# violetdenim/c3dgs

Hardware: AMD Instinct MI355X
Metric: raster views/sec fwd+bwd @1920x1080 (higher is better)
Workload: dtype f32; 1 GPU; BASELINE.json configs[2]: synth-v1 3M Gaussians, SH deg 3, indexed-camera rasterizer (QAT inner loop), mark_visible+fwd+bwd, 1 view/step/GPU; gaussians=3000000, width=1920, height=1080, sh_codebook=304096, gaussian_codebook=754096, parallelism=replicas x1

## Files before the change

### c3dgs_amd/_lib.py

```python
import ctypes as C
import os

import torch

_HERE = os.path.dirname(os.path.abspath(__file__))
LIB_PATH = os.environ.get("C3DGS_LIB_PATH") or os.path.join(_HERE, "libc3dgs_hip.so")

_f32p = C.POINTER(C.c_float)
_i64p = C.POINTER(C.c_int64)
_i32p = C.POINTER(C.c_int32)
_u8p = C.POINTER(C.c_uint8)

RESIZE_FN = C.CFUNCTYPE(C.c_void_p, C.c_void_p, C.c_size_t)


class RasterParams(C.Structure):
    _fields_ = [
        ("P", C.c_int32), ("D", C.c_int32), ("M", C.c_int32), ("W", C.c_int32), ("H", C.c_int32),
        ("SHS", C.c_int32), ("GS", C.c_int32),
        ("background", C.c_void_p), ("means3D", C.c_void_p), ("sh", C.c_void_p), ("colors_precomp", C.c_void_p),
        ("opacities", C.c_void_p), ("scales", C.c_void_p), ("scale_factors", C.c_void_p), ("rotations", C.c_void_p),
        ("cov3D_precomp", C.c_void_p), ("sh_indices", C.c_void_p), ("g_indices", C.c_void_p),
        ("viewmatrix", C.c_void_p), ("projmatrix", C.c_void_p), ("campos", C.c_void_p),
        ("tan_fovx", C.c_float), ("tan_fovy", C.c_float), ("scale_modifier", C.c_float),
# ... 126 lines not shown
    "c3dgs_ray_fill_xyz": (C.c_int, [C.c_int32, _vp, _vp, _vp, C.c_float, C.c_int64, _vp, _vp, _vp, _vp, _vp]),
    "c3dgs_image_from_u8": (C.c_int, [C.c_int32, C.c_int32, C.c_int32, _vp, C.c_int32, _vp, C.c_int32, C.c_int32, _vp, _vp]),
    "c3dgs_adam_step": (C.c_int, [C.c_int32, C.POINTER(AdamTensor), C.c_double, C.c_double, C.c_double, _vp]),
    "c3dgs_sparse_adam_workspace_bytes": (C.c_int, [C.c_int64, C.POINTER(C.c_size_t)]),
    "c3dgs_sparse_adam_select": (C.c_int, [C.c_int64, _vp, C.c_int32, _vp, _vp]),
    "c3dgs_sparse_adam_step": (C.c_int, [C.c_int32, C.POINTER(SparseAdamTensor), C.c_int64, _vp, C.c_double, C.c_double, C.c_double,
                                         _vp]),
    "c3dgs_densify_classify": (C.c_int, [C.c_int32] + [_vp] * 7 + [C.c_float] * 4 + [_vp, _vp]),
    "c3dgs_rows_plan_workspace_bytes": (C.c_size_t, [C.c_int32]),
    "c3dgs_rows_plan": (C.c_int, [C.c_int32, _vp, C.c_int32, C.c_int64, _vp, _vp, _vp, _vp, _vp, _vp]),
    "c3dgs_rows_apply": (C.c_int, [C.c_int32, C.c_int64, _vp, _vp, _vp, C.c_int32, C.POINTER(RowsTensor), C.c_int32, C.c_int64,
                                   _vp, _vp, _vp, C.c_int32, C.c_int32, _vp]),
    "c3dgs_densify_stats": (C.c_int, [C.c_int32] + [_vp] * 7),
    "c3dgs_mcmc_workspace_bytes": (C.c_int, [C.c_int64, C.POINTER(C.c_size_t)]),
    "c3dgs_mcmc_sample": (C.c_int, [C.c_int64, _vp, _vp, C.c_int32, C.c_float, _vp, C.c_int64, _vp, C.c_int32, _vp, _vp, _vp, _vp,
                                    _vp, _vp]),
    "c3dgs_mcmc_apply": (C.c_int, [C.c_int64, C.c_int64, _vp, C.c_int64, _vp, _vp, C.c_int32, C.POINTER(RowsTensor), C.c_int32,
                                   C.c_float, _vp, _vp]),
    "c3dgs_mcmc_noise": (C.c_int, [C.c_int64] + [_vp] * 6 + [C.c_float, C.c_float, _vp]),
    "c3dgs_bilagrid_workspace_bytes": (C.c_size_t, [C.c_int32] * 5),
    "c3dgs_bilagrid_slice": (C.c_int, [C.c_int32] * 5 + [_vp] * 4),
    "c3dgs_bilagrid_slice_backward": (C.c_int, [C.c_int32] * 5 + [_vp] * 7),
    "c3dgs_bilagrid_tv": (C.c_int, [C.c_int32] * 4 + [_vp] * 4),
    "c3dgs_bilagrid_tv_backward": (C.c_int, [C.c_int32] * 4 + [_vp] * 4),
    "c3dgs_index_plan_workspace_bytes": (C.c_size_t, [C.c_int32, C.c_int32, C.c_int32]),
    "c3dgs_index_plan": (C.c_int, [C.c_int32, _vp, _vp, C.c_int32, _vp, C.c_int32, C.c_int64, C.c_int64, C.c_int64] + [_vp] * 8),
    "c3dgs_extract_rot_scale": (C.c_int, [C.c_int32, _vp, _vp, _vp, _vp]),
    "c3dgs_l1_ssim_forward": (C.c_int, [C.c_int32, C.c_int32, C.c_int32, C.c_void_p, C.c_void_p, C.c_void_p, C.c_void_p,
                                        C.c_void_p]),
    "c3dgs_l1_ssim_value": (C.c_int, [C.c_void_p, C.c_double, C.c_double, C.c_double, C.c_void_p, C.c_void_p]),
    "c3dgs_l1_ssim_backward": (C.c_int, [C.c_int32, C.c_int32, C.c_int32, C.c_void_p, C.c_void_p, C.c_void_p, C.c_void_p,
                                         C.c_float, C.c_float, C.c_void_p, C.c_void_p]),
    "c3dgs_image_metrics_ws_bytes": (C.c_size_t, [C.c_int32, C.c_int32, C.c_int32, C.c_int32]),
    "c3dgs_image_metrics": (C.c_int, [C.c_int32, C.c_int32, C.c_int32, C.c_int32, _vp, _vp, _vp, C.c_size_t, _vp, _vp]),
    "c3dgs_qat_workspace_bytes": (C.c_size_t, []),
    "c3dgs_qat_scan_bytes": (C.c_size_t, [C.c_int32]),
    "c3dgs_qat_observe": (C.c_int, [C.POINTER(QatParams), _vp, _vp]),
    "c3dgs_qat_codebooks": (C.c_int, [C.POINTER(QatParams), _vp, _vp, _vp, _vp]),
    "c3dgs_qat_codebooks_backward": (C.c_int, [C.POINTER(QatParams)] + [_vp] * 8),
    "c3dgs_qat_visible": (C.c_int, [C.POINTER(QatParams), _vp, _vp, _vp, _vp, _vp, _vp]),
    "c3dgs_qat_points": (C.c_int, [C.POINTER(QatParams)] + [_vp] * 10),
    "c3dgs_qat_points_backward": (C.c_int, [C.POINTER(QatParams)] + [_vp] * 11),
    "c3dgs_qat_quantize": (C.c_int, [C.POINTER(QatParams), C.c_int32] + [_vp] * 7),
    "c3dgs_fake_quantize": (C.c_int, [C.c_int64, _vp, _vp, C.c_int32, C.c_int32, C.c_float, _vp, _vp, _vp]),
    "c3dgs_fake_quantize_backward": (C.c_int, [C.c_int64, _vp, _vp, C.c_int32, _vp, _vp, _vp]),
    "c3dgs_debug_sort_temp_bytes": (C.c_size_t, [C.c_int32, C.c_int64, C.c_int32]),
    "c3dgs_debug_sort_pairs": (C.c_int, [C.c_int32, C.c_int64, C.c_int32, _vp, _vp, _vp, _vp, _vp, C.c_size_t, _vp]),
    "c3dgs_debug_tile_sort_temp_bytes": (C.c_size_t, [C.c_int32, C.c_int64]),
    "c3dgs_debug_tile_sort_pairs": (C.c_int, [C.c_int32, C.c_int64, _vp, _vp, _vp, _vp, _vp, C.c_size_t, _vp]),
    "c3dgs_get_geom_layout": (C.c_int, [C.c_int32, C.POINTER(GeomLayout)]),
    "c3dgs_get_binning_layout": (C.c_int, [C.c_int32, C.c_int32, C.c_int32, C.POINTER(BinningLayout)]),
    "c3dgs_get_image_layout": (C.c_int, [C.c_int32, C.c_int32, C.POINTER(ImageLayout)]),
    "c3dgs_get_compact_layout": (C.c_int, [C.c_int32, C.c_int32, C.c_int32, C.POINTER(CompactLayout)]),
    "c3dgs_get_backward_layout": (C.c_int, [C.c_int32, C.c_int32, C.POINTER(BackwardLayout)]),
    "c3dgs_backward_workspace_bytes": (C.c_size_t, [C.c_int32, C.c_int32]),
    "c3dgs_profile_enable": (C.c_int, [C.c_int]),
    "c3dgs_profile_only": (C.c_int, [C.c_char_p]),
    "c3dgs_profile_read": (C.c_int, [C.POINTER(StageTime), C.c_int]),
    "c3dgs_last_error": (C.c_char_p, []),
    "c3dgs_abi_version": (C.c_int, []),
    "c3dgs_abs_accumulate": (C.c_int, [C.c_int64, C.c_void_p, C.c_void_p, C.c_void_p]),
}
DIAG_PROTOTYPES = {
    "c3dgs_debug_lane_counters": (C.c_int, [C.POINTER(C.c_uint64), _vp]),
    "c3dgs_debug_sort_times": (C.c_int, [C.POINTER(C.c_uint64)]),
    "c3dgs_debug_gather_probe": (C.c_int, [C.c_int32, C.c_int64, _vp, _vp, _vp, _vp]),
}

_lib = None


def lib():
    global _lib
    if _lib is None:
        if not os.path.exists(LIB_PATH):
            raise RuntimeError(
                f"c3dgs_amd: {LIB_PATH} is missing. Build it with `python -m c3dgs_amd.build` "
                "(hipcc --offload-arch=gfx950). There is no CPU fallback for this package.")
        try:
            handle = C.CDLL(LIB_PATH)
        except OSError as e:
            raise RuntimeError(f"c3dgs_amd: cannot load {LIB_PATH}: {e}") from e
        diag = {n: p for n, p in DIAG_PROTOTYPES.items() if hasattr(handle, n)}
        for name, (res, args) in {**PROTOTYPES, **diag}.items():
            fn = getattr(handle, name)
            fn.restype = res
            fn.argtypes = args
        _lib = handle
    return _lib


def check(rc):
    if rc != 0:
        msg = lib().c3dgs_last_error()
        raise RuntimeError((msg or b"unknown error").decode("utf-8", "replace"))


def stream(device):
    return C.c_void_p(torch.cuda.current_stream(device).cuda_stream)


def ptr(t):
    return None if t is None else t.data_ptr()


def gpu_tensor(t, name, dtype=torch.float32):
# ... 29 lines not shown
```

### c3dgs_amd/csrc/c_abi.hip

```cpp
#include "common.hpp"
#include "mcmc.hpp"
#include "bilagrid.hpp"
#include <cfloat>
#include <climits>
#include <cstdlib>
#include <cstring>
#include <mutex>
#include <vector>

namespace c3dgs {

static thread_local std::string g_last_error;
void set_error(const std::string& msg) { g_last_error = msg; }

#define C3DGS_STAGE_TABLE(X)                                                                                                   \
    X(MARK_VISIBLE, "mark_visible") X(PREPROCESS, "preprocess") X(DEPTH_SORT, "depth_sort") X(SCAN, "scan")                    \
    X(DUPLICATE, "duplicate_with_keys") X(SORT, "sort") X(RANGES, "identify_ranges") X(RENDER_FWD, "render_forward")           \
    X(RENDER_DEPTH, "render_depth")                                                                                            \
    X(RENDER_CONTRIB, "render_contrib") X(RENDER_CONTRIB_BLEND, "render_contrib_blend") X(RENDER_CONTRIB_SUM, "render_contrib_sum") \
    X(RENDER_ERROR, "render_error") X(RENDER_ERROR_BLEND, "render_error_blend") X(RENDER_ERROR_SUM, "render_error_sum")           \
    X(ERROR_MAP_L1, "error_map_l1")                                                                                            \
    X(POSE_GRAD, "pose_grad") X(POSE_GRAD_SUMS, "pose_grad_sums") X(POSE_GRAD_FOLD, "pose_grad_fold")                          \
    X(ZERO_PARTIALS, "zero_partials") X(RENDER_BWD, "render_backward") X(BWD_PREPROCESS, "backward_preprocess")                \
    X(RENDER_DEPTH_BWD, "render_depth_backward") X(DEPTH_BWD_FOLD, "depth_backward_fold")                                      \
// ... 349 lines not shown
    for (auto& r : recs) {
        float ms = 0.f;
        if (hipEventSynchronize(r.b) == hipSuccess && hipEventElapsedTime(&ms, r.a, r.b) == hipSuccess) {
            total[r.stage] += (double)ms;
            count[r.stage]++;
        }
    }
    {
        std::lock_guard<std::mutex> lk(g_prof_mu);
        for (auto& r : recs) { g_prof_pool.push_back(r.a); g_prof_pool.push_back(r.b); }
    }
    int n = 0;
    for (int i = 0; i < ST_COUNT && n < capacity; i++) {
        if (!count[i]) continue;
        std::memset(&out[n], 0, sizeof(out[n]));
        std::strncpy(out[n].name, kStageNames[i], sizeof(out[n].name) - 1);
        out[n].total_ms = total[i];
        out[n].count = count[i];
        n++;
    }
    return n;
}
int c3dgs_abi_version(void) { return C3DGS_ABI_VERSION; }

int c3dgs_get_geom_layout(int32_t P, c3dgs_geom_layout* out)
{
    if (!out || P < 0) return fail(C3DGS_E_INVALID, "bad arguments");
    geom_layout(P, out);
    return C3DGS_OK;
}
int c3dgs_get_binning_layout(int32_t R, int32_t W, int32_t H, c3dgs_binning_layout* out)
{
    if (!out || R < 0 || W <= 0 || H <= 0) return fail(C3DGS_E_INVALID, "bad arguments");
    binning_layout(R, W, H, out);
    return C3DGS_OK;
}
int c3dgs_get_image_layout(int32_t W, int32_t H, c3dgs_image_layout* out)
{
    if (!out || W <= 0 || H <= 0) return fail(C3DGS_E_INVALID, "bad arguments");
    ImageLayout L; image_layout(W, H, &L);
    *out = L;
    return C3DGS_OK;
}
int c3dgs_get_compact_layout(int32_t R, int32_t W, int32_t H, c3dgs_compact_layout* out)
{
    if (!out || R < 0 || W <= 0 || H <= 0) return fail(C3DGS_E_INVALID, "bad arguments");
    c3dgs_binning_layout BL; binning_layout(R, W, H, &BL);
    const CompactBinLayout C = compact_bin_layout(R);
    ImageLayout IL; image_layout(W, H, &IL);
    out->cqm = BL.sort_temp + C.cqm; out->cid = BL.sort_temp + C.cid;
    out->tile_used_c = IL.tile_used_c; out->n_contrib_c = IL.n_contrib_c;
    return C3DGS_OK;
}
int c3dgs_get_backward_layout(int32_t P, int32_t R, c3dgs_backward_layout* out)
{
    if (!out || P < 0 || R < 0) return fail(C3DGS_E_INVALID, "bad arguments");
    backward_layout(P, R, out);
    return C3DGS_OK;
}
size_t c3dgs_backward_workspace_bytes(int32_t P, int32_t R)
{
    c3dgs_backward_layout L; backward_layout(P, R, &L);
    return L.total_bytes;
}

int c3dgs_mark_visible(int32_t P, const float* means3D, const float* viewmatrix, const float* projmatrix, uint8_t* present,
                       void* stream)
{
    (void)projmatrix;
    if (P < 0) return fail(C3DGS_E_INVALID, "P must be >= 0");
    if (P == 0) return C3DGS_OK;
    if (!means3D || !viewmatrix || !present) return fail(C3DGS_E_INVALID, "means3D, viewmatrix and present are required");
    C3DGS_TIMED_STAGE(ST_MARK_VISIBLE, 0, (hipStream_t)stream, launch_mark_visible(P, means3D, viewmatrix, present, (hipStream_t)stream));
    return C3DGS_OK;
}

int c3dgs_mark_visible_pose(int32_t P, const float* means3D, const float* extrinsic_vector, uint8_t* present, void* stream)
{
    if (P < 0) return fail(C3DGS_E_INVALID, "P must be >= 0");
    if (P == 0) return C3DGS_OK;
    if (!means3D || !extrinsic_vector || !present) return fail(C3DGS_E_INVALID, "means3D, extrinsic_vector and present are required");
    C3DGS_TIMED_STAGE(ST_MARK_VISIBLE, 0, (hipStream_t)stream, launch_mark_visible_pose(P, means3D, extrinsic_vector, present, (hipStream_t)stream));
    return C3DGS_OK;
}

int c3dgs_camera_from_pose(const float* extrinsic_vector, float inv_tan_half_fovx, float inv_tan_half_fovy, float* viewmatrix,
                           float* projmatrix, float* campos, void* stream)
{
    if (!extrinsic_vector || !viewmatrix || !projmatrix || !campos) return fail(C3DGS_E_INVALID, "camera_from_pose: NULL pointer");
    launch_camera_from_pose(extrinsic_vector, inv_tan_half_fovx, inv_tan_half_fovy, viewmatrix, projmatrix, campos, (hipStream_t)stream);
    C3DGS_STAGE("camera_from_pose", 0, (hipStream_t)stream);
    return C3DGS_OK;
}

int c3dgs_rasterize_gaussians(const c3dgs_raster_params* p, c3dgs_resize_fn geom_resize, void* geom_user,
                              c3dgs_resize_fn binning_resize, void* binning_user, c3dgs_resize_fn image_resize,
                              void* image_user, float* out_color, int32_t* radii, int32_t* num_rendered, void* stream)
{
    return forward_impl(p, false, geom_resize, geom_user, binning_resize, binning_user, image_resize, image_user, out_color,
                        radii, num_rendered, stream);
}

int c3dgs_rasterize_gaussians_indexed(const c3dgs_raster_params* p, c3dgs_resize_fn geom_resize, void* geom_user,
                                      c3dgs_resize_fn binning_resize, void* binning_user, c3dgs_resize_fn image_resize,
                                      void* image_user, float* out_color, int32_t* radii, int32_t* num_rendered, void* stream)
{
// ... 987 lines not shown
```

### c3dgs_amd/csrc/common.hpp

```cpp
#pragma once
#include <hip/hip_runtime.h>
#include <cstdint>
#include <cstddef>
#include <cstdio>
#include <cstring>
#include <string>

#include "../../include/c3dgs_hip.h"

namespace c3dgs {

constexpr int TILE = 16;
constexpr int TILE_PIX = 256;
constexpr int SPLAT_F4 = 3;
constexpr int PARTIAL_FLOATS = 9;
constexpr int BWD_LIST = 1024;

void set_error(const std::string& msg);
inline int fail(int code, const std::string& msg) { set_error(msg); return code; }

#define C3DGS_HIP_TRY(expr)                                                                         \
    do {                                                                                            \
        hipError_t e__ = (expr);                                                                    \
        if (e__ != hipSuccess)                                                                      \
// ... 33 lines not shown
{
    uint32_t msb = sizeof(n) * 4, step = msb;
    while (step > 1) {
        step /= 2;
        if (n >> msb) msb += step; else msb -= step;
    }
    if (n >> msb) msb++;
    return msb;
}

inline void geom_layout(int P, c3dgs_geom_layout* L)
{
    size_t o = 0, p = (size_t)(P > 0 ? P : 1);
    L->splat = o;             o = align_up(o + p * SPLAT_F4 * 16);
    L->depth_keys = o;        o = align_up(o + p * 4);
    L->depth_keys_sorted = o; o = align_up(o + p * 4);
    L->depth_order = o;       o = align_up(o + p * 4);
    L->sorted_offsets = o;    o = align_up(o + p * 8);
    L->inst_offset = o;       o = align_up(o + p * 4);
    L->rects = o;             o = align_up(o + p * 8);
    L->clamped = o;           o = align_up(o + p);
    L->block_base = o;        o = align_up(o + ((p + 255) / 256 + 2) * 4);
    L->depth_base = o;        o = align_up(o + ((p + 255) / 256 + 1) * 4);
    L->scan_temp = o;         L->scan_temp_bytes = scan_temp_bytes((int)p);
    o = align_up(o + L->scan_temp_bytes);
    L->total_bytes = o;
}

inline size_t geom_gtab_bytes(const c3dgs_raster_params& p) { return (p.g_indices && p.scales) ? align_up((size_t)(p.GS > 0 ? p.GS : 1) * 32) : 0; }

inline int tile_key_bytes_for(long long T) { return T > 65536 ? 4 : 2; }
inline int tile_key_bytes(int W, int H) { return tile_key_bytes_for((long long)tiles_x(W) * tiles_y(H)); }
inline int tile_sort_end_bit_for(long long T)
{
    const int msb = (int)higher_msb((uint32_t)T), kbits = 8 * tile_key_bytes_for(T);
    return msb < kbits ? msb : kbits;
}
inline int tile_sort_end_bit(int W, int H) { return tile_sort_end_bit_for((long long)tiles_x(W) * tiles_y(H)); }

inline void binning_layout(int R, int W, int H, c3dgs_binning_layout* L)
{
    size_t o = 0, r = (size_t)(R > 0 ? R : 1);
    const int end_bit = tile_sort_end_bit(W, H);
    const size_t kb = (size_t)tile_key_bytes(W, H);
    L->keys_unsorted = o;   o = align_up(o + r * kb);
    L->values_unsorted = o; o = align_up(o + r * 4);
    L->keys_sorted = o;     o = align_up(o + r * kb);
    L->point_list = o;      o = align_up(o + r * 4);
    L->sort_temp = o;       L->sort_temp_bytes = sort_temp_bytes((int)r, end_bit, (int)kb);
    o = align_up(o + L->sort_temp_bytes);
    L->total_bytes = o;
}

struct ImageLayout : c3dgs_image_layout { size_t tile_used_c, n_contrib_c; };
inline void image_layout(int W, int H, ImageLayout* L)
{
    size_t o = 0, n = (size_t)W * H, t = (size_t)tiles_x(W) * tiles_y(H);
    L->final_T = o;     o = align_up(o + n * 4);
    L->n_contrib = o;   o = align_up(o + n * 4);
    L->ranges = o;      o = align_up(o + t * 8);
    L->tile_used = o;   o = align_up(o + t * 4);
    L->tile_order = o;  o = align_up(o + t * 4);
    L->tile_used_c = o; o = align_up(o + t * 4);
    L->n_contrib_c = o; o = align_up(o + n * 4);
    L->total_bytes = o;
}

struct CompactBinLayout { size_t cqm, cid, bin_bytes; };
inline CompactBinLayout compact_bin_layout(int R)
{
    const size_t r = (size_t)(R > 0 ? R : 1);
    CompactBinLayout C;
    C.cqm = 0; C.cid = align_up(r); C.bin_bytes = C.cid + align_up(r * 4);
    return C;
}

inline void backward_layout(int P, int R, c3dgs_backward_layout* L)
{
    size_t o = 0, r = (size_t)(R > 0 ? R : 1), n_lists = ((size_t)(P > 0 ? P : 1) + BWD_LIST - 1) / BWD_LIST;
    L->partials = o;   o = align_up(o + r * PARTIAL_FLOATS * sizeof(float));
    L->touched = o;    o = align_up(o + r);
    L->live_ids = o;   o = align_up(o + n_lists * BWD_LIST * 4);
    L->live_slots = o; o = align_up(o + n_lists * BWD_LIST * 4);
    L->live_count = o; o = align_up(o + n_lists * 4);
    L->list_len = BWD_LIST;
    L->total_bytes = o;
}

struct DepthBackwardLayout { size_t dz, total_bytes; };
inline DepthBackwardLayout depth_backward_layout(int P, int R)
{
    c3dgs_backward_layout B; backward_layout(P, R, &B);
    const size_t r = (size_t)(R > 0 ? R : 1);
    DepthBackwardLayout L;
    L.dz = B.total_bytes;
    L.total_bytes = align_up(L.dz + r * sizeof(float));
    return L;
}

struct ContribSlot { float sum, max; uint32_t hits; };
struct ContribLayout { size_t slots, touched, touched_bytes, total_bytes; };
inline ContribLayout contrib_layout(int P, int R)
{
    (void)P;
    size_t o = 0, r = (size_t)(R > 0 ? R : 1);
    ContribLayout L;
    L.slots = o;   o = align_up(o + r * sizeof(ContribSlot));
    L.touched = o; o = align_up(o + r);
    L.touched_bytes = o - L.touched;
    L.total_bytes = o;
    return L;
}

struct ErrorLayout { size_t slots, touched, touched_bytes, total_bytes; };
inline ErrorLayout error_layout(int P, int R)
{
    (void)P;
    size_t o = 0, r = (size_t)(R > 0 ? R : 1);
    ErrorLayout L;
    L.slots = o;   o = align_up(o + r * sizeof(float));
    L.touched = o; o = align_up(o + r);
    L.touched_bytes = o - L.touched;
    L.total_bytes = o;
    return L;
}

constexpr int SPARSE_ADAM_SELECT_ROWS = 256;
struct SparseAdamLayout { size_t count, rows, block_base, total_bytes; };
inline SparseAdamLayout sparse_adam_layout(int64_t P)
{
    const size_t p = (size_t)(P > 0 ? P : 1);
    SparseAdamLayout L;
    size_t o = 0;
    L.count = o;      o = align_up(o + 4);
    L.rows = o;       o = align_up(o + p * 4);
    L.block_base = o; o = align_up(o + ((p + SPARSE_ADAM_SELECT_ROWS - 1) / SPARSE_ADAM_SELECT_ROWS + 2) * 4);
    L.total_bytes = o;
    return L;
}

struct GeomPtrs {
    float4* splat; uint32_t* depth_keys; uint32_t* depth_keys_sorted;
    uint32_t* depth_order; uint2* sorted_offsets; uint32_t* inst_offset; uint16_t* rects;
    uint8_t* clamped; uint32_t* block_base; uint32_t* depth_base; void* scan_temp; size_t scan_temp_bytes;
    float4* gtab;
};
struct BinPtrs {
    void* keys_unsorted; uint32_t* values_unsorted; void* keys_sorted; uint32_t* point_list;
    void* sort_temp; size_t sort_temp_bytes; int key_bytes;
};
struct ImgPtrs { float* final_T; uint32_t* n_contrib; uint2* ranges; uint32_t* tile_used; uint32_t* tile_order;
                 uint32_t* tile_used_c; uint32_t* n_contrib_c; };
struct CompactPtrs { uint8_t* cqm; uint32_t* cid; };
struct BwdPtrs { float* partials; uint8_t* touched; size_t touched_bytes;
                 uint32_t* live_ids; uint32_t* live_slots; uint32_t* live_count; };
struct ContribPtrs { ContribSlot* slots; uint8_t* touched; size_t touched_bytes; };
struct ErrorPtrs { float* slots; uint8_t* touched; size_t touched_bytes; };

inline GeomPtrs geom_ptrs(void* base, int P)
{
    c3dgs_geom_layout L; geom_layout(P, &L);
    char* b = (char*)base;
    return { (float4*)(b + L.splat), (uint32_t*)(b + L.depth_keys), (uint32_t*)(b + L.depth_keys_sorted), (uint32_t*)(b + L.depth_order),
             (uint2*)(b + L.sorted_offsets), (uint32_t*)(b + L.inst_offset), (uint16_t*)(b + L.rects),
             (uint8_t*)(b + L.clamped), (uint32_t*)(b + L.block_base), (uint32_t*)(b + L.depth_base), (void*)(b + L.scan_temp),
             L.scan_temp_bytes, (float4*)(b + L.total_bytes) };
}
inline BinPtrs bin_ptrs(void* base, int R, int W, int H)
{
    c3dgs_binning_layout L; binning_layout(R, W, H, &L);
    char* b = (char*)base;
    return { (void*)(b + L.keys_unsorted), (uint32_t*)(b + L.values_unsorted), (void*)(b + L.keys_sorted),
             (uint32_t*)(b + L.point_list), (void*)(b + L.sort_temp), L.sort_temp_bytes, tile_key_bytes(W, H) };
}
inline ImgPtrs img_ptrs(void* base, int W, int H)
{
    ImageLayout L; image_layout(W, H, &L);
    char* b = (char*)base;
    return { (float*)(b + L.final_T), (uint32_t*)(b + L.n_contrib), (uint2*)(b + L.ranges), (uint32_t*)(b + L.tile_used),
             (uint32_t*)(b + L.tile_order), (uint32_t*)(b + L.tile_used_c), (uint32_t*)(b + L.n_contrib_c) };
}
inline CompactPtrs compact_ptrs(const BinPtrs& bp, int R)
{
    const CompactBinLayout C = compact_bin_layout(R);
    return { (uint8_t*)bp.sort_temp + C.cqm, (uint32_t*)((char*)bp.sort_temp + C.cid) };
}
inline BwdPtrs bwd_ptrs(void* base, int P, int R)
{
    c3dgs_backward_layout L; backward_layout(P, R, &L);
    char* b = (char*)base;
    return { (float*)(b + L.partials), (uint8_t*)(b + L.touched), L.live_ids - L.touched,
             (uint32_t*)(b + L.live_ids), (uint32_t*)(b + L.live_slots), (uint32_t*)(b + L.live_count) };
}

inline ContribPtrs contrib_ptrs(void* base, int P, int R)
{
    const ContribLayout L = contrib_layout(P, R);
    char* b = (char*)base;
    return { (ContribSlot*)(b + L.slots), (uint8_t*)(b + L.touched), L.touched_bytes };
}

inline ErrorPtrs error_ptrs(void* base, int P, int R)
{
    const ErrorLayout L = error_layout(P, R);
    char* b = (char*)base;
    return { (float*)(b + L.slots), (uint8_t*)(b + L.touched), L.touched_bytes };
}

void launch_camera_from_pose(const float* pose, float inv_tan_x, float inv_tan_y, float* view, float* proj, float* campos, hipStream_t s);
void launch_mark_visible(int P, const float* means3D, const float* view, uint8_t* present, hipStream_t s);
void launch_mark_visible_pose(int P, const float* means3D, const float* pose7, uint8_t* present, hipStream_t s);
void launch_pack_codebook(const c3dgs_raster_params& p, float4* gtab, hipStream_t s);
void launch_preprocess(const c3dgs_raster_params& p, const GeomPtrs& g, int32_t* radii, uint2* ranges, void* zero_span, size_t zero_n16,
                       hipStream_t s);
void launch_scan_blocks(int nb, uint32_t* base, const uint32_t* sort_err, uint32_t* host_out, uint32_t host_seq, hipStream_t s);
void launch_depth_order_scan(int P, const GeomPtrs& g, hipStream_t s);
void launch_duplicate_with_keys(int P, const GeomPtrs& g, const BinPtrs& b, int grid_x, const uint32_t* sort_err,
                                void* zero_span, size_t zero_n16, hipStream_t s);
void launch_identify_ranges(int R, const void* keys_sorted, int key_bytes, uint2* ranges, const uint32_t* sort_err, hipStream_t s);
hipError_t run_depth_sort(void* temp, size_t temp_bytes, const uint32_t* kin, uint32_t* kout, const uint32_t* vin,
                          uint32_t* vout, int P, const uint2* rects, uint2* rects_sorted, hipStream_t s, bool ctrl_cleared = false,
                          bool rects_fit_bytes = false, bool hist_done = false);
hipError_t run_depth_hist_scan(void* temp, size_t temp_bytes, const uint32_t* keys, int P, int nb, uint32_t* base,
                               const uint32_t* sort_err, uint32_t* host_out, uint32_t host_seq, hipStream_t s);
hipError_t run_tile_sort(void* temp, size_t temp_bytes, const void* kin, void* kout, int key_bytes, const uint32_t* vin,
                         uint32_t* vout, int R, int end_bit, hipStream_t s, bool ctrl_cleared = false);
size_t depth_sort_clear_bytes(int P);
size_t tile_sort_clear_bytes(int R, int end_bit, int key_bytes);
bool onesweep_enabled();
int onesweep_timed_out(hipStream_t s);
uint32_t* onesweep_error_word();
size_t onesweep_depth_temp_bytes(int P);
size_t onesweep_tile_temp_bytes(int R, int end_bit, int key_bytes = 2);
// ... 136 lines not shown
```

### c3dgs_amd/csrc/render.hip

```cpp
#include "common.hpp"
#include "render_diag.hpp"
#include "render_common.hpp"
#include <algorithm>

namespace c3dgs {

__global__ void __launch_bounds__(1024) backward_prep_kernel(int T, const uint32_t* __restrict__ tile_used, uint32_t* __restrict__ order,
                                                              uint4* __restrict__ zero_a, size_t n16_a, uint4* __restrict__ zero_b, size_t n16_b)
{
    if (blockIdx.x > 0) {
        const uint4 z = make_uint4(0u, 0u, 0u, 0u);
        const size_t stride = (size_t)(gridDim.x - 1) * 1024;
        for (size_t i = (size_t)(blockIdx.x - 1) * 1024 + threadIdx.x; i < n16_a; i += stride) zero_a[i] = z;
        for (size_t i = (size_t)(blockIdx.x - 1) * 1024 + threadIdx.x; i < n16_b; i += stride) zero_b[i] = z;
        return;
    }
    if (T <= 0) return;
    auto work = [&](int i) { return tile_used[i]; };
    __shared__ uint32_t s_cnt[1024], s_w[16];
    const int t = threadIdx.x, lane = t & 63, wave = t >> 6;
    s_cnt[t] = 0;
    __syncthreads();
    for (int i = t; i < T; i += 1024) atomicAdd(&s_cnt[1023 - min(work(i) >> 3, 1023u)], 1u);
    __syncthreads();
    const uint32_t c = s_cnt[t];
    uint32_t incl = c;
#pragma unroll
    for (int o = 1; o < 64; o <<= 1) { const uint32_t v = __shfl_up(incl, o); if (lane >= o) incl += v; }
    if (lane == 63) s_w[wave] = incl;
    __syncthreads();
    uint32_t off = 0;
    for (int w = 0; w < wave; w++) off += s_w[w];
    s_cnt[t] = off + incl - c;
    __syncthreads();
    for (int i = t; i < T; i += 1024) order[atomicAdd(&s_cnt[1023 - min(work(i) >> 3, 1023u)], 1u)] = (uint32_t)i;
}

__global__ void __launch_bounds__(256)
render_forward_kernel(int W, int H, int gx, int T, const uint2* __restrict__ ranges, const uint32_t* __restrict__ point_list,
                      const float4* __restrict__ splat, const float* __restrict__ bg, float* __restrict__ out_color,
                      float* __restrict__ final_T, uint32_t* __restrict__ n_contrib, uint32_t* __restrict__ tile_used,
                      uint32_t* __restrict__ n_contrib_c, uint32_t* __restrict__ tile_used_c, uint8_t* __restrict__ cqm,
                      uint32_t* __restrict__ cid, const uint32_t* __restrict__ sort_err)
{
    const int tile = tile_of_block(blockIdx.x, T);
    if (tile >= T || (blockIdx.x >> 3) >= ((T + 7) >> 3)) return;
    __shared__ float4 s_ab[2][BATCH + 1][2];
    __shared__ float s_c[2][BATCH + 1];
    __shared__ uint32_t s_list[4][BATCH + 8];
    __shared__ int s_wdone[2][4];
    __shared__ unsigned long long s_mask[2][4][4];
    __shared__ __attribute__((aligned(4))) uint8_t s_live[2][4];
    __shared__ uint32_t s_used, s_used_c;
    static_assert(sizeof(s_ab) + sizeof(s_c) + sizeof(s_list) + sizeof(s_wdone) + sizeof(s_mask) + sizeof(s_live) + 2 * sizeof(uint32_t)
                      <= 18 * 1280, "render_forward: more than 18 LDS granules = six workgroups per CU instead of seven");
    constexpr uint32_t REC_BYTES = 32, BUF_BYTES = (BATCH + 1) * REC_BYTES;

    const int tid = threadIdx.x, wave = tid >> 6, lane = tid & 63;
    const int tx = tile % gx, ty = tile / gx;
    const int px = tx * TILE + (wave & 1) * 8 + (lane & 7);
    const int py = ty * TILE + (wave >> 1) * 8 + (lane >> 3);
    const bool inside = px < W && py < H;
    const float pxf = (float)px, pyf = (float)py;
    bool done = !inside;
    if (tid == 0) { s_used = 0; s_used_c = 0; }
    if (tid < 2) { s_ab[tid][BATCH][0] = make_float4(0, 0, 0, 0); s_ab[tid][BATCH][1] = make_float4(0, 0, 0, 0); s_c[tid][BATCH] = 0.f; }
    const float tile_x0 = (float)(tx * TILE), tile_y0 = (float)(ty * TILE);

    const bool poisoned = *sort_err != 0u;
    const uint2 range = poisoned ? make_uint2(0u, 0u) : ranges[tile];
    const int n = (int)(range.y - range.x);
    const int rounds = (n + BATCH - 1) / BATCH;

    float Tr = 1.0f, C0 = 0.f, C1 = 0.f, C2 = 0.f;
    uint32_t last_contributor = 0, last_contributor_c = 0;
    uint32_t n_live = 0;
    constexpr uint32_t NO_ENTRY = 0xffffffffu;
    LaneCount lc;
    const char* rec_base = reinterpret_cast<const char*>(&s_ab[0][0][0]);
    const char* blue_base = reinterpret_cast<const char*>(&s_c[0][0]);

    float4 ra = make_float4(0, 0, 0, 0), rb = ra, rc = ra;
    uint32_t id = 0u;
    if (tid < n) {
        id = point_list[range.x + tid];
        ra = splat[3 * (size_t)id]; rb = splat[3 * (size_t)id + 1]; rc = splat[3 * (size_t)id + 2];
    }
    for (int r = 0; r < rounds; r++) {
// ... 113 lines not shown
{
    return __int_as_float(__builtin_amdgcn_update_dpp(0, __float_as_int(v), CTRL, 0xf, 0xf, true));
}

template <int N, int CTRL>
__device__ __forceinline__ void transpose_reduce_step(float* v, bool hi)
{
#pragma unroll
    for (int k = 0; k < N / 2; k++) {
        const float keep = hi ? v[k + N / 2] : v[k];
        const float send = hi ? v[k] : v[k + N / 2];
        v[k] = keep + dpp_take<CTRL>(send);
    }
}

#define C3DGS_TR4(CTRL, LO, HI, o, a, b, base, half)                                                                      \
    asm volatile("s_nop 1\n\t"                                                                                            \
                 "v_add_f32_dpp %0, %4, %4 " CTRL " row_mask:0xf bank_mask:" LO "\n\t"                                    \
                 "v_add_f32_dpp %1, %5, %5 " CTRL " row_mask:0xf bank_mask:" LO "\n\t"                                    \
                 "v_add_f32_dpp %2, %6, %6 " CTRL " row_mask:0xf bank_mask:" LO "\n\t"                                    \
                 "v_add_f32_dpp %3, %7, %7 " CTRL " row_mask:0xf bank_mask:" LO "\n\t"                                    \
                 "v_add_f32_dpp %0, %8, %8 " CTRL " row_mask:0xf bank_mask:" HI "\n\t"                                    \
                 "v_add_f32_dpp %1, %9, %9 " CTRL " row_mask:0xf bank_mask:" HI "\n\t"                                    \
                 "v_add_f32_dpp %2, %10, %10 " CTRL " row_mask:0xf bank_mask:" HI "\n\t"                                  \
                 "v_add_f32_dpp %3, %11, %11 " CTRL " row_mask:0xf bank_mask:" HI                                         \
                 : "=&v"(o[base]), "=&v"(o[base + 1]), "=&v"(o[base + 2]), "=&v"(o[base + 3])                             \
                 : "v"(a[base]), "v"(a[base + 1]), "v"(a[base + 2]), "v"(a[base + 3]), "v"(b[base + half]),               \
                   "v"(b[base + half + 1]), "v"(b[base + half + 2]), "v"(b[base + half + 3]))

__device__ __forceinline__ void reduce_columns_24(float* u, int lane)
{
    transpose_reduce_step<24, 0xB1>(u, (lane & 1) != 0);
    transpose_reduce_step<12, 0x4E>(u, (lane & 2) != 0);
}

__device__ __forceinline__ void reduce_rows_9(const float* n, float& total, float& ninth)
{
    float o[4];
    C3DGS_TR4("row_ror:8", "0x3", "0xc", o, n, n, 0, 4);
    float t8;
    asm volatile("s_nop 1\n\tv_add_f32_dpp %0, %1, %1 row_ror:8 row_mask:0xf bank_mask:0xf" : "=&v"(t8) : "v"(n[8]));
    auto s0 = __builtin_amdgcn_permlane16_swap(__float_as_uint(o[0]), __float_as_uint(o[2]), false, false);
    auto s1 = __builtin_amdgcn_permlane16_swap(__float_as_uint(o[1]), __float_as_uint(o[3]), false, false);
    auto s8 = __builtin_amdgcn_permlane16_swap(__float_as_uint(t8), __float_as_uint(t8), false, false);
    const float w0 = __uint_as_float(s0[0]) + __uint_as_float(s0[1]);
    const float w1 = __uint_as_float(s1[0]) + __uint_as_float(s1[1]);
    const float w8 = __uint_as_float(s8[0]) + __uint_as_float(s8[1]);
    auto s2 = __builtin_amdgcn_permlane32_swap(__float_as_uint(w0), __float_as_uint(w1), false, false);
    auto s9 = __builtin_amdgcn_permlane32_swap(__float_as_uint(w8), __float_as_uint(w8), false, false);
    total = __uint_as_float(s2[0]) + __uint_as_float(s2[1]);
    ninth = __uint_as_float(s9[0]) + __uint_as_float(s9[1]);
}

#ifndef C3DGS_BWD_WPE
#define C3DGS_BWD_WPE 5
#endif
__global__ void __launch_bounds__(256) __attribute__((amdgpu_waves_per_eu(C3DGS_BWD_WPE, C3DGS_BWD_WPE)))
render_backward_kernel(int W, int H, int gx, int T, const uint2* __restrict__ ranges, const uint32_t* __restrict__ tile_used_c,
                       const uint32_t* __restrict__ cid, const float4* __restrict__ splat,
                       const uint32_t* __restrict__ block_base, const float* __restrict__ bg, const float* __restrict__ final_Ts,
                       const uint32_t* __restrict__ n_contrib_c, const float* __restrict__ dL_dpixels,
                       float* __restrict__ partials, uint8_t* __restrict__ touched, const uint8_t* __restrict__ cqm,
                       const uint32_t* __restrict__ tile_order, uint4* __restrict__ zero_span, size_t zero_n16)
{
    if (zero_n16) {
        const size_t per = (zero_n16 + gridDim.x - 1) / gridDim.x, z0 = (size_t)blockIdx.x * per, z1 = min(z0 + per, zero_n16);
        for (size_t i = z0 + threadIdx.x; i < z1; i += 256) zero_span[i] = make_uint4(0u, 0u, 0u, 0u);
    }
    if ((int)blockIdx.x >= T) return;
    PhaseClock clk;
    const int tile = (int)tile_order[blockIdx.x];
    __shared__ float4 s_ab[BATCH + 1][2];
    __shared__ float s_c[BATCH + 1];
    __shared__ uint32_t s_slot[BATCH];
    __shared__ uint32_t s_list[4][BATCH / 2 + GROUP_G];
    __shared__ unsigned long long s_mask[4][4];
    __shared__ float s_part[2][BATCH][NPART];
    constexpr uint32_t REC_BYTES = 32;
    const char* rec_base = reinterpret_cast<const char*>(&s_ab[0][0]);
    const char* blue_base = reinterpret_cast<const char*>(&s_c[0]);

    const int tid = threadIdx.x, wave = tid >> 6, lane = tid & 63;
    const int tx = tile % gx, ty = tile / gx;
    const int px = tx * TILE + (wave & 1) * 8 + (lane & 7);
    const int py = ty * TILE + (wave >> 1) * 8 + (lane >> 3);
    const bool inside = px < W && py < H;
    const float pxf = (float)px, pyf = (float)py;
    const size_t pix = (size_t)W * py + px, HW = (size_t)H * W;

    const uint2 range = ranges[tile];
    const int n = (int)(range.y - range.x);
    const int used = min(n, (int)tile_used_c[tile]);
    if (used <= 0) return;
    const int rounds = (used + BATCH - 1) / BATCH;
    if (tid == 0) { s_ab[BATCH][0] = make_float4(0, 0, 0, 0); s_ab[BATCH][1] = make_float4(0, 0, 0, 0); s_c[BATCH] = 0.f; }
    for (int q = tid; q < 4 * (BATCH / 2 + GROUP_G); q += 256) (&s_list[0][0])[q] = (uint32_t)BATCH * REC_BYTES;

    const float T_final = inside ? final_Ts[pix] : 0.f;
    float Tr = T_final;
    const int last_contributor = inside ? (int)n_contrib_c[pix] : 0;
    float dpx0 = 0.f, dpx1 = 0.f, dpx2 = 0.f;
    if (inside) { dpx0 = dL_dpixels[pix]; dpx1 = dL_dpixels[HW + pix]; dpx2 = dL_dpixels[2 * HW + pix]; }
    float Sd = T_final * (bg[0] * dpx0 + bg[1] * dpx1 + bg[2] * dpx2);
    int wave_last = last_contributor;
#pragma unroll
    for (int o = 32; o > 0; o >>= 1) wave_last = max(wave_last, __shfl_xor(wave_last, o));
    wave_last = __builtin_amdgcn_readfirstlane(wave_last);
    const int beta = candidate_of_lane(lane);
    const int my_m = ((lane >> 3) & 1) * 4 + ((lane >> 4) & 1) * 2 + ((lane >> 5) & 1);
    LaneCount lc;

    uint32_t next_id = 0u, next_qm = 0u;
    {
        const int p0 = used - 1 - tid;
        if (p0 >= 0) { next_id = cid[range.x + p0]; next_qm = cqm[range.x + p0]; }
    }
    clk.mark(PhaseClock::PROLOGUE);
    for (int r = 0; r < rounds; r++) {
        __syncthreads();
        clk.mark(PhaseClock::TOP_BARRIER);
        const int mypos = used - 1 - (r * BATCH + tid);
        uint32_t qm = 0u;
        if (mypos >= 0) {
            const uint32_t id = next_id;
            qm = next_qm;
            float4 a = splat[3 * (size_t)id], b = splat[3 * (size_t)id + 1];
            const float4 c = splat[3 * (size_t)id + 2];
            prescale_conic(a, b);
            s_slot[tid] = entry_slot(c, block_base, id, tx, ty);
            s_ab[tid][0] = a; s_ab[tid][1] = b; s_c[tid] = c.x;
        }
        {
            const int npos = mypos - BATCH;
            if (npos >= 0) { next_id = cid[range.x + npos]; next_qm = cqm[range.x + npos]; }
        }
#pragma unroll
        for (int q = 0; q < 4; q++) {
            const unsigned long long bm = __ballot((qm >> q) & 1u);
            if (lane == 0) s_mask[q][wave] = bm;
        }
        clk.mark(PhaseClock::GATHER);
#pragma unroll
        for (int w = 0; w < 2; w++)
#pragma unroll
            for (int q = 0; q < NPART; q++) s_part[w][tid][q] = 0.f;
        clk.mark(PhaseClock::CLEAR);
        __syncthreads();
        clk.mark(PhaseClock::CLOSE_BARRIER);

        const int cnt = min(BATCH, used - r * BATCH);
        const int pos0 = used - 1 - r * BATCH;
        const int thr = (pos0 - last_contributor) * (int)REC_BYTES;
#pragma unroll 1
        for (int half = 0; half < 2; half++) {
        int nw = 0;
        {
            const unsigned long long lt = (1ull << lane) - 1ull;
#pragma unroll
            for (int cc = 0; cc < 2; cc++) {
                const int c = half * 2 + cc;
                unsigned long long m = uniform_u64(s_mask[wave][c]);
                const int jmin = pos0 - wave_last + 1 - c * 64;
                if (jmin >= 64) m = 0; else if (jmin > 0) m &= ~0ull << jmin;
                if ((m >> lane) & 1ull) s_list[wave][nw + (int)__popcll(m & lt)] = (uint32_t)(c * 64 + lane) * REC_BYTES;
                nw += (int)__popcll(m);
            }
            if (lane < GROUP_G) s_list[wave][nw + lane] = (uint32_t)BATCH * REC_BYTES;
            __builtin_amdgcn_fence(__ATOMIC_RELEASE, "wavefront");
            __builtin_amdgcn_wave_barrier();
            __builtin_amdgcn_fence(__ATOMIC_ACQUIRE, "wavefront");
        }
        clk.mark(PhaseClock::COMPACT);
        uint4 row0 = *reinterpret_cast<const uint4*>(&s_list[wave][0]);
        uint4 row1 = *reinterpret_cast<const uint4*>(&s_list[wave][4]);
        float4 a_n = *reinterpret_cast<const float4*>(rec_base + row0.x);
        float4 b_n = *reinterpret_cast<const float4*>(rec_base + row0.x + 16);
        float c_n = *reinterpret_cast<const float*>(blue_base + (row0.x >> 3));
        for (int k = 0; k < nw; k += GROUP_G) {
            const uint32_t* lrow = &s_list[wave][k];
            const uint32_t e[GROUP_G] = { row0.x, row0.y, row0.z, row0.w, row1.x, row1.y, row1.z, row1.w };
            float v[GROUP_G * NCOL];
            float u[GROUP_G * NCOL / 2];
            const uint32_t my_off = lrow[beta];
#pragma unroll
            for (int g = 0; g < GROUP_G; g++) {
                const float4 a = a_n, b = b_n;
                const float cblue = c_n;
// ... 12 lines not shown
                Tr = Tr * rinv;
                const float dchannel_dcolor = a_eff * Tr;
                const float cd = fmaf(cblue, dpx2, fmaf(b.w, dpx1, b.z * dpx0));
                v[g * NCOL + 0] = dchannel_dcolor * dpx0;
                v[g * NCOL + 1] = dchannel_dcolor * dpx1;
                v[g * NCOL + 2] = dchannel_dcolor * dpx2;
                const float dL_dalpha = fmaf(Tr, cd, -(rinv * Sd));
                Sd = fmaf(dchannel_dcolor, cd, Sd);
                const float w = G_eff * dL_dalpha, wx = w * dx;
                v[g * NCOL + 3] = w;
                v[g * NCOL + 4] = wx;
                v[g * NCOL + 5] = wx * dx;
                if (g == 4) { C3DGS_TR4("row_half_mirror", "0x5", "0xa", u, v, v, 0, 24); }
                if (g == 5) { C3DGS_TR4("row_half_mirror", "0x5", "0xa", u, v, v, 4, 24); C3DGS_TR4("row_half_mirror", "0x5", "0xa", u, v, v, 8, 24); }
                if (g == 6) { C3DGS_TR4("row_half_mirror", "0x5", "0xa", u, v, v, 12, 24); }
                if (g == 7) { C3DGS_TR4("row_half_mirror", "0x5", "0xa", u, v, v, 16, 24); C3DGS_TR4("row_half_mirror", "0x5", "0xa", u, v, v, 20, 24); }
            }
            row0 = *reinterpret_cast<const uint4*>(lrow + GROUP_G);
            row1 = *reinterpret_cast<const uint4*>(lrow + GROUP_G + 4);
            reduce_columns_24(u, lane);
            a_n = *reinterpret_cast<const float4*>(rec_base + row0.x);
            b_n = *reinterpret_cast<const float4*>(rec_base + row0.x + 16);
            c_n = *reinterpret_cast<const float*>(blue_base + (row0.x >> 3));
            const int myj = (int)(my_off >> 5);
            const float dyb = *reinterpret_cast<const float*>(rec_base + my_off + 4) - pyf;
            float total, ninth;
            const float nine[NPART] = { u[0], u[1], u[2], u[3], u[4], u[5], dyb * u[3], dyb * u[4], (dyb * dyb) * u[3] };
            reduce_rows_9(nine, total, ninth);
            if (myj < BATCH) {
                __hip_atomic_fetch_add(&s_part[wave >> 1][myj][my_m], total, __ATOMIC_RELAXED, __HIP_MEMORY_SCOPE_WORKGROUP);
                if (lane < 8) __hip_atomic_fetch_add(&s_part[wave >> 1][myj][8], ninth, __ATOMIC_RELAXED, __HIP_MEMORY_SCOPE_WORKGROUP);
            }
        }
        lc.end_list();
        __builtin_amdgcn_fence(__ATOMIC_RELEASE, "wavefront");
        __builtin_amdgcn_wave_barrier();
        clk.mark(PhaseClock::GROUPS);
        }
        __syncthreads();
        clk.mark(PhaseClock::FLUSH_BARRIER);
        if (tid < cnt) {
            const uint32_t slot = s_slot[tid];
            float* dst = partials + (size_t)slot * NPART;
            float t[NPART];
#pragma unroll
            for (int q = 0; q < NPART; q++) t[q] = s_part[0][tid][q] + s_part[1][tid][q];
            dst[0] = t[0]; dst[1] = t[1]; dst[2] = t[2];
            dst[3] = t[3]; dst[4] = t[4]; dst[5] = t[6];
            dst[6] = t[5]; dst[7] = t[7]; dst[8] = t[8];
            touched[slot] = 1;
        }
        clk.mark(PhaseClock::FLUSH_STORES);
    }
    lc.flush(8, lane);
    clk.flush(lane);
}

void launch_backward_prep(int W, int H, const ImgPtrs& img, void* zero_a, size_t n16_a, void* zero_b, size_t n16_b, hipStream_t s)
{
    const int T = (W > 0 && H > 0) ? tiles_x(W) * tiles_y(H) : 0;
    const size_t n16 = n16_a + n16_b;
    if (T <= 0 && n16 == 0) return;
    const unsigned fill = n16 ? (unsigned)std::min<size_t>((n16 + 1023) / 1024, 1024) : 0u;
    backward_prep_kernel<<<1 + fill, 1024, 0, s>>>(T, img.tile_used_c, img.tile_order, (uint4*)zero_a, n16_a, (uint4*)zero_b, n16_b);
}

void launch_render_backward(int W, int H, const ImgPtrs& img, const float4* splat,
                            const uint32_t* block_base, const float* bg, const float* dL_dpix, float* partials,
                            uint8_t* touched, const CompactPtrs& cl, void* zero_span, size_t zero_n16, hipStream_t s)
{
    const int gx = tiles_x(W), T = gx * tiles_y(H);
    render_backward_kernel<<<banded_grid(T), 256, 0, s>>>(W, H, gx, T, img.ranges, img.tile_used_c, cl.cid, splat, block_base, bg, img.final_T,
                                                img.n_contrib_c, dL_dpix, partials, touched, cl.cqm, img.tile_order, (uint4*)zero_span,
                                                zero_span ? zero_n16 : 0);
}

}
```

### include/c3dgs_hip.h

```cpp
#ifndef C3DGS_HIP_H
#define C3DGS_HIP_H

#include <stddef.h>
#include <stdint.h>

#ifdef __cplusplus
extern "C" {
#endif

#define C3DGS_ABI_VERSION 4

enum {
    C3DGS_OK = 0,
    C3DGS_E_INVALID = 1,
    C3DGS_E_HIP = 2,
    C3DGS_E_ALLOC = 3
};

typedef void* (*c3dgs_resize_fn)(void* user, size_t bytes);

typedef struct c3dgs_raster_params {
    int32_t P;
    int32_t D;
    int32_t M;
// ... 336 lines not shown
    size_t depth_order;
    size_t sorted_offsets;
    size_t inst_offset;
    size_t rects;
    size_t clamped;
    size_t scan_temp;
    size_t scan_temp_bytes;
    size_t block_base;
    size_t depth_base;
} c3dgs_geom_layout;

typedef struct c3dgs_binning_layout {
    size_t total_bytes;
    size_t keys_unsorted;
    size_t values_unsorted;
    size_t keys_sorted;
    size_t point_list;
    size_t sort_temp;
    size_t sort_temp_bytes;
} c3dgs_binning_layout;

typedef struct c3dgs_image_layout {
    size_t total_bytes;
    size_t final_T;
    size_t n_contrib;
    size_t ranges;
    size_t tile_used;
    size_t tile_order;
} c3dgs_image_layout;

int c3dgs_get_geom_layout(int32_t P, c3dgs_geom_layout* out);
int c3dgs_get_binning_layout(int32_t R, int32_t W, int32_t H, c3dgs_binning_layout* out);
typedef struct c3dgs_backward_layout {
    size_t total_bytes;
    size_t partials;
    size_t touched;
    size_t live_ids;
    size_t live_slots;
    size_t live_count;
    size_t list_len;
} c3dgs_backward_layout;

int c3dgs_get_image_layout(int32_t W, int32_t H, c3dgs_image_layout* out);
int c3dgs_get_backward_layout(int32_t P, int32_t R, c3dgs_backward_layout* out);
size_t c3dgs_backward_workspace_bytes(int32_t P, int32_t R);

typedef struct c3dgs_compact_layout {
    size_t cqm;
    size_t cid;
    size_t tile_used_c;
    size_t n_contrib_c;
} c3dgs_compact_layout;
int c3dgs_get_compact_layout(int32_t R, int32_t W, int32_t H, c3dgs_compact_layout* out);

typedef struct c3dgs_stage_time {
    char name[32];
    double total_ms;
    int64_t count;
} c3dgs_stage_time;
int c3dgs_profile_enable(int on);
int c3dgs_profile_only(const char* stage_name);
int c3dgs_profile_read(c3dgs_stage_time* out, int capacity);

const char* c3dgs_last_error(void);
int c3dgs_abi_version(void);

#ifdef __cplusplus
}
#endif
#endif
```

Baseline: 638.2 views/s.

## Precompute per-tile descriptors in backward prep to shorten render-backward prologue

The backward prep kernel now writes a 16-byte descriptor per sorted tile holding the tile id, range start and used count. Render-backward reads this with one load instead of a dependent chain of tile_order, ranges and tile_used_c lookups. The zero-fill slice moves to the end of the block so it stops delaying the tile's work, and the first cid/cqm prefetch is issued earlier. It also adds a DPP wave max and pins uniform values in scalar registers, at the cost of an extra image-layout buffer and extra prep-kernel stores.

```diff
diff --git a/c3dgs_amd/_lib.py b/c3dgs_amd/_lib.py
--- a/c3dgs_amd/_lib.py
+++ b/c3dgs_amd/_lib.py
@@ -202,6 +202,7 @@
     "c3dgs_get_binning_layout": (C.c_int, [C.c_int32, C.c_int32, C.c_int32, C.POINTER(BinningLayout)]),
     "c3dgs_get_image_layout": (C.c_int, [C.c_int32, C.c_int32, C.POINTER(ImageLayout)]),
     "c3dgs_get_compact_layout": (C.c_int, [C.c_int32, C.c_int32, C.c_int32, C.POINTER(CompactLayout)]),
+    "c3dgs_get_tile_desc_offset": (C.c_int, [C.c_int32, C.c_int32, C.POINTER(C.c_size_t)]),
     "c3dgs_get_backward_layout": (C.c_int, [C.c_int32, C.c_int32, C.POINTER(BackwardLayout)]),
     "c3dgs_backward_workspace_bytes": (C.c_size_t, [C.c_int32, C.c_int32]),
     "c3dgs_profile_enable": (C.c_int, [C.c_int]),
diff --git a/c3dgs_amd/csrc/c_abi.hip b/c3dgs_amd/csrc/c_abi.hip
--- a/c3dgs_amd/csrc/c_abi.hip
+++ b/c3dgs_amd/csrc/c_abi.hip
@@ -425,6 +425,13 @@
     out->tile_used_c = IL.tile_used_c; out->n_contrib_c = IL.n_contrib_c;
     return C3DGS_OK;
 }
+int c3dgs_get_tile_desc_offset(int32_t W, int32_t H, size_t* out)
+{
+    if (!out || W <= 0 || H <= 0) return fail(C3DGS_E_INVALID, "bad arguments");
+    ImageLayout IL; image_layout(W, H, &IL);
+    *out = IL.tile_desc;
+    return C3DGS_OK;
+}
 int c3dgs_get_backward_layout(int32_t P, int32_t R, c3dgs_backward_layout* out)
 {
     if (!out || P < 0 || R < 0) return fail(C3DGS_E_INVALID, "bad arguments");
diff --git a/c3dgs_amd/csrc/common.hpp b/c3dgs_amd/csrc/common.hpp
--- a/c3dgs_amd/csrc/common.hpp
+++ b/c3dgs_amd/csrc/common.hpp
@@ -109,7 +109,7 @@
     L->total_bytes = o;
 }
 
-struct ImageLayout : c3dgs_image_layout { size_t tile_used_c, n_contrib_c; };
+struct ImageLayout : c3dgs_image_layout { size_t tile_used_c, n_contrib_c, tile_desc; };
 inline void image_layout(int W, int H, ImageLayout* L)
 {
     size_t o = 0, n = (size_t)W * H, t = (size_t)tiles_x(W) * tiles_y(H);
@@ -117,6 +117,7 @@
     L->n_contrib = o;   o = align_up(o + n * 4);
     L->ranges = o;      o = align_up(o + t * 8);
     L->tile_used = o;   o = align_up(o + t * 4);
+    L->tile_desc = o;   o = align_up(o + t * 16);
     L->tile_order = o;  o = align_up(o + t * 4);
     L->tile_used_c = o; o = align_up(o + t * 4);
     L->n_contrib_c = o; o = align_up(o + n * 4);
@@ -207,7 +208,7 @@
     void* sort_temp; size_t sort_temp_bytes; int key_bytes;
 };
 struct ImgPtrs { float* final_T; uint32_t* n_contrib; uint2* ranges; uint32_t* tile_used; uint32_t* tile_order;
-                 uint32_t* tile_used_c; uint32_t* n_contrib_c; };
+                 uint32_t* tile_used_c; uint32_t* n_contrib_c; uint4* tile_desc; };
 struct CompactPtrs { uint8_t* cqm; uint32_t* cid; };
 struct BwdPtrs { float* partials; uint8_t* touched; size_t touched_bytes;
                  uint32_t* live_ids; uint32_t* live_slots; uint32_t* live_count; };
@@ -235,7 +236,8 @@
     ImageLayout L; image_layout(W, H, &L);
     char* b = (char*)base;
     return { (float*)(b + L.final_T), (uint32_t*)(b + L.n_contrib), (uint2*)(b + L.ranges), (uint32_t*)(b + L.tile_used),
-             (uint32_t*)(b + L.tile_order), (uint32_t*)(b + L.tile_used_c), (uint32_t*)(b + L.n_contrib_c) };
+             (uint32_t*)(b + L.tile_order), (uint32_t*)(b + L.tile_used_c), (uint32_t*)(b + L.n_contrib_c),
+             (uint4*)(b + L.tile_desc) };
 }
 inline CompactPtrs compact_ptrs(const BinPtrs& bp, int R)
 {
diff --git a/c3dgs_amd/csrc/render.hip b/c3dgs_amd/csrc/render.hip
--- a/c3dgs_amd/csrc/render.hip
+++ b/c3dgs_amd/csrc/render.hip
@@ -5,7 +5,8 @@
 
 namespace c3dgs {
 
-__global__ void __launch_bounds__(1024) backward_prep_kernel(int T, const uint32_t* __restrict__ tile_used, uint32_t* __restrict__ order,
+__global__ void __launch_bounds__(1024) backward_prep_kernel(int T, const uint32_t* __restrict__ tile_used, const uint2* __restrict__ ranges,
+                                                              uint32_t* __restrict__ order, uint4* __restrict__ desc,
                                                               uint4* __restrict__ zero_a, size_t n16_a, uint4* __restrict__ zero_b, size_t n16_b)
 {
     if (blockIdx.x > 0) {
@@ -16,12 +17,23 @@
         return;
     }
     if (T <= 0) return;
-    auto work = [&](int i) { return tile_used[i]; };
     __shared__ uint32_t s_cnt[1024], s_w[16];
     const int t = threadIdx.x, lane = t & 63, wave = t >> 6;
+    constexpr int KEEP = 8;
+    uint32_t wk[KEEP];
+    uint2 rk[KEEP];
+#pragma unroll
+    for (int k = 0; k < KEEP; k++) {
+        const int i = min(t + k * 1024, T - 1);
+        wk[k] = tile_used[i]; rk[k] = ranges[i];
+    }
+    auto bucket = [](uint32_t w) { return 1023 - (int)min(w >> 3, 1023u); };
     s_cnt[t] = 0;
     __syncthreads();
-    for (int i = t; i < T; i += 1024) atomicAdd(&s_cnt[1023 - min(work(i) >> 3, 1023u)], 1u);
+#pragma unroll
+    for (int k = 0; k < KEEP; k++)
+        if (t + k * 1024 < T) atomicAdd(&s_cnt[bucket(wk[k])], 1u);
+    for (int i = t + KEEP * 1024; i < T; i += 1024) atomicAdd(&s_cnt[bucket(tile_used[i])], 1u);
     __syncthreads();
     const uint32_t c = s_cnt[t];
     uint32_t incl = c;
@@ -33,7 +45,15 @@
     for (int w = 0; w < wave; w++) off += s_w[w];
     s_cnt[t] = off + incl - c;
     __syncthreads();
-    for (int i = t; i < T; i += 1024) order[atomicAdd(&s_cnt[1023 - min(work(i) >> 3, 1023u)], 1u)] = (uint32_t)i;
+    auto place = [&](int i, uint32_t w, uint2 range) {
+        const uint32_t b = atomicAdd(&s_cnt[bucket(w)], 1u);
+        order[b] = (uint32_t)i;
+        desc[b] = make_uint4((uint32_t)i, range.x, (uint32_t)min((int)(range.y - range.x), (int)w), 0u);
+    };
+#pragma unroll
+    for (int k = 0; k < KEEP; k++)
+        if (t + k * 1024 < T) place(t + k * 1024, wk[k], rk[k]);
+    for (int i = t + KEEP * 1024; i < T; i += 1024) place(i, tile_used[i], ranges[i]);
 }
 
 __global__ void __launch_bounds__(256)
@@ -253,24 +273,43 @@
     ninth = __uint_as_float(s9[0]) + __uint_as_float(s9[1]);
 }
 
+__device__ __forceinline__ int wave_max_i32(int v)
+{
+    v = max(v, __builtin_amdgcn_update_dpp(v, v, 0xB1, 0xf, 0xf, false));
+    v = max(v, __builtin_amdgcn_update_dpp(v, v, 0x4E, 0xf, 0xf, false));
+    v = max(v, __builtin_amdgcn_update_dpp(v, v, 0x141, 0xf, 0xf, false));
+    v = max(v, __builtin_amdgcn_update_dpp(v, v, 0x140, 0xf, 0xf, false));
+    return max(max(__builtin_amdgcn_readlane(v, 0), __builtin_amdgcn_readlane(v, 16)),
+               max(__builtin_amdgcn_readlane(v, 32), __builtin_amdgcn_readlane(v, 48)));
+}
+
 #ifndef C3DGS_BWD_WPE
 #define C3DGS_BWD_WPE 5
 #endif
 __global__ void __launch_bounds__(256) __attribute__((amdgpu_waves_per_eu(C3DGS_BWD_WPE, C3DGS_BWD_WPE)))
-render_backward_kernel(int W, int H, int gx, int T, const uint2* __restrict__ ranges, const uint32_t* __restrict__ tile_used_c,
+render_backward_kernel(int W, int H, int gx, int T, const uint4* __restrict__ tile_desc,
                        const uint32_t* __restrict__ cid, const float4* __restrict__ splat,
                        const uint32_t* __restrict__ block_base, const float* __restrict__ bg, const float* __restrict__ final_Ts,
                        const uint32_t* __restrict__ n_contrib_c, const float* __restrict__ dL_dpixels,
                        float* __restrict__ partials, uint8_t* __restrict__ touched, const uint8_t* __restrict__ cqm,
-                       const uint32_t* __restrict__ tile_order, uint4* __restrict__ zero_span, size_t zero_n16)
-{
-    if (zero_n16) {
-        const size_t per = (zero_n16 + gridDim.x - 1) / gridDim.x, z0 = (size_t)blockIdx.x * per, z1 = min(z0 + per, zero_n16);
-        for (size_t i = z0 + threadIdx.x; i < z1; i += 256) zero_span[i] = make_uint4(0u, 0u, 0u, 0u);
-    }
-    if ((int)blockIdx.x >= T) return;
+                       uint4* __restrict__ zero_span, size_t zero_n16)
+{
+    auto clear_slice = [&]() {
+        if (zero_n16) {
+            const size_t per = (zero_n16 + gridDim.x - 1) / gridDim.x, z0 = (size_t)blockIdx.x * per, z1 = min(z0 + per, zero_n16);
+            for (size_t i = z0 + threadIdx.x; i < z1; i += 256) zero_span[i] = make_uint4(0u, 0u, 0u, 0u);
+        }
+    };
+    if ((int)blockIdx.x >= T) { clear_slice(); return; }
     PhaseClock clk;
-    const int tile = (int)tile_order[blockIdx.x];
+    const uint4 desc = tile_desc[blockIdx.x];
+    const float bg0 = bg[0], bg1 = bg[1], bg2 = bg[2];
+    const int tile = (int)desc.x;
+    const uint32_t range_x = desc.y;
+    const int used = (int)desc.z;
+    asm volatile("" :: "s"(cid), "s"(cqm), "s"(final_Ts), "s"(n_contrib_c), "s"(dL_dpixels), "s"(tile), "s"(range_x), "s"(used),
+                 "s"(bg0), "s"(bg1), "s"(bg2));
+    if (used <= 0) { clear_slice(); return; }
     __shared__ float4 s_ab[BATCH + 1][2];
     __shared__ float s_c[BATCH + 1];
     __shared__ uint32_t s_slot[BATCH];
@@ -288,34 +327,29 @@
     const bool inside = px < W && py < H;
     const float pxf = (float)px, pyf = (float)py;
     const size_t pix = (size_t)W * py + px, HW = (size_t)H * W;
-
-    const uint2 range = ranges[tile];
-    const int n = (int)(range.y - range.x);
-    const int used = min(n, (int)tile_used_c[tile]);
-    if (used <= 0) return;
     const int rounds = (used + BATCH - 1) / BATCH;
-    if (tid == 0) { s_ab[BATCH][0] = make_float4(0, 0, 0, 0); s_ab[BATCH][1] = make_float4(0, 0, 0, 0); s_c[BATCH] = 0.f; }
-    for (int q = tid; q < 4 * (BATCH / 2 + GROUP_G); q += 256) (&s_list[0][0])[q] = (uint32_t)BATCH * REC_BYTES;
-
+
+    uint32_t next_id = 0u, next_qm = 0u;
+    {
+        const int p0 = used - 1 - tid;
+        if (p0 >= 0) { next_id = cid[range_x + p0]; next_qm = cqm[range_x + p0]; }
+    }
     const float T_final = inside ? final_Ts[pix] : 0.f;
-    float Tr = T_final;
     const int last_contributor = inside ? (int)n_contrib_c[pix] : 0;
     float dpx0 = 0.f, dpx1 = 0.f, dpx2 = 0.f;
     if (inside) { dpx0 = dL_dpixels[pix]; dpx1 = dL_dpixels[HW + pix]; dpx2 = dL_dpixels[2 * HW + pix]; }
-    float Sd = T_final * (bg[0] * dpx0 + bg[1] * dpx1 + bg[2] * dpx2);
-    int wave_last = last_contributor;
-#pragma unroll
-    for (int o = 32; o > 0; o >>= 1) wave_last = max(wave_last, __shfl_xor(wave_last, o));
-    wave_last = __builtin_amdgcn_readfirstlane(wave_last);
+    __builtin_amdgcn_sched_barrier(0);
+
+    if (tid == 0) { s_ab[BATCH][0] = make_float4(0, 0, 0, 0); s_ab[BATCH][1] = make_float4(0, 0, 0, 0); s_c[BATCH] = 0.f; }
+    for (int q = tid; q < 4 * (BATCH / 2 + GROUP_G); q += 256) (&s_list[0][0])[q] = (uint32_t)BATCH * REC_BYTES;
+
+    float Tr = T_final;
+    float Sd = T_final * (bg0 * dpx0 + bg1 * dpx1 + bg2 * dpx2);
+    const int wave_last = wave_max_i32(last_contributor);
     const int beta = candidate_of_lane(lane);
     const int my_m = ((lane >> 3) & 1) * 4 + ((lane >> 4) & 1) * 2 + ((lane >> 5) & 1);
     LaneCount lc;
 
-    uint32_t next_id = 0u, next_qm = 0u;
-    {
-        const int p0 = used - 1 - tid;
-        if (p0 >= 0) { next_id = cid[range.x + p0]; next_qm = cqm[range.x + p0]; }
-    }
     clk.mark(PhaseClock::PROLOGUE);
     for (int r = 0; r < rounds; r++) {
         __syncthreads();
@@ -333,7 +367,7 @@
         }
         {
             const int npos = mypos - BATCH;
-            if (npos >= 0) { next_id = cid[range.x + npos]; next_qm = cqm[range.x + npos]; }
+            if (npos >= 0) { next_id = cid[range_x + npos]; next_qm = cqm[range_x + npos]; }
         }
 #pragma unroll
         for (int q = 0; q < 4; q++) {
@@ -452,6 +486,7 @@
         }
         clk.mark(PhaseClock::FLUSH_STORES);
     }
+    clear_slice();
     lc.flush(8, lane);
     clk.flush(lane);
 }
@@ -462,7 +497,8 @@
     const size_t n16 = n16_a + n16_b;
     if (T <= 0 && n16 == 0) return;
     const unsigned fill = n16 ? (unsigned)std::min<size_t>((n16 + 1023) / 1024, 1024) : 0u;
-    backward_prep_kernel<<<1 + fill, 1024, 0, s>>>(T, img.tile_used_c, img.tile_order, (uint4*)zero_a, n16_a, (uint4*)zero_b, n16_b);
+    backward_prep_kernel<<<1 + fill, 1024, 0, s>>>(T, img.tile_used_c, img.ranges, img.tile_order, img.tile_desc, (uint4*)zero_a, n16_a,
+                                                   (uint4*)zero_b, n16_b);
 }
 
 void launch_render_backward(int W, int H, const ImgPtrs& img, const float4* splat,
@@ -470,8 +506,8 @@
                             uint8_t* touched, const CompactPtrs& cl, void* zero_span, size_t zero_n16, hipStream_t s)
 {
     const int gx = tiles_x(W), T = gx * tiles_y(H);
-    render_backward_kernel<<<banded_grid(T), 256, 0, s>>>(W, H, gx, T, img.ranges, img.tile_used_c, cl.cid, splat, block_base, bg, img.final_T,
-                                                img.n_contrib_c, dL_dpix, partials, touched, cl.cqm, img.tile_order, (uint4*)zero_span,
+    render_backward_kernel<<<banded_grid(T), 256, 0, s>>>(W, H, gx, T, img.tile_desc, cl.cid, splat, block_base, bg, img.final_T,
+                                                img.n_contrib_c, dL_dpix, partials, touched, cl.cqm, (uint4*)zero_span,
                                                 zero_span ? zero_n16 : 0);
 }
 
diff --git a/include/c3dgs_hip.h b/include/c3dgs_hip.h
--- a/include/c3dgs_hip.h
+++ b/include/c3dgs_hip.h
@@ -412,6 +412,7 @@
     size_t n_contrib_c;
 } c3dgs_compact_layout;
 int c3dgs_get_compact_layout(int32_t R, int32_t W, int32_t H, c3dgs_compact_layout* out);
+int c3dgs_get_tile_desc_offset(int32_t W, int32_t H, size_t* out);
 
 typedef struct c3dgs_stage_time {
     char name[32];
```

Result: no change. 640.0 views/s (median of 2 runs) (+0.3%).
